# ApsaraDB/galaxysql

Measured on AMD Instinct MI355X. Metric: probe_rows_per_s, higher is better.
Workload: dtype int64; 1 GPU; C3_tpch_sf100_q3_join_chain_groupby; customer_rows_per_gpu=15000000, orders_rows_per_gpu=150000000, lineitem_rows_scanned_per_gpu=600000000, lineitem_rows_joined_per_gpu=323601457, groups_last_step=12883243, aggregates=SUM(revenue) f64 + SUM(rev_scaled4) i64 + COUNT(*), exchange=none, parallelism=hash_shuffle_dp1, probe_launches=81

## Files before the change

galaxysql_amd/abi.py:

```python
from __future__ import annotations

import ctypes as C
import os

import numpy as np

from .chunk import (Block, Chunk, I64, I32, F64, SLICE, DECIMAL,
                    _NP_DTYPES)

_REPO = os.path.dirname(os.path.dirname(os.path.abspath(__file__)))


class GxBlock(C.Structure):
    _fields_ = [
        ("type", C.c_int32),
        ("mem", C.c_int32),
        ("values", C.c_void_p),
        ("nulls", C.c_void_p),
        ("offsets", C.c_void_p),
        ("data", C.c_void_p),
        ("data_len", C.c_int64),
    ]


# ... 322 lines not shown
        L.gxop_window_close.argtypes = [C.c_void_p]
        L.gxop_fwindow_create.restype = C.c_void_p
        L.gxop_fwindow_create.argtypes = [C.POINTER(GxFWindowCfg)]
        L.gxop_fwindow_consume.argtypes = [C.c_void_p, C.POINTER(GxChunk)]
        L.gxop_fwindow_finish.argtypes = [C.c_void_p]
        L.gxop_fwindow_next.argtypes = [C.c_void_p,
                                        C.POINTER(C.POINTER(GxResult))]
        L.gxop_fwindow_close.argtypes = [C.c_void_p]
        L.gxop_part_create.restype = C.c_void_p
        L.gxop_part_create.argtypes = [C.POINTER(GxPartCfg)]
        L.gxop_part_consume.argtypes = [C.c_void_p, C.POINTER(GxChunk),
                                        C.POINTER(C.POINTER(GxResult))]
        L.gxop_part_consume_concat.argtypes = [C.c_void_p, C.POINTER(GxChunk),
                                               C.POINTER(C.POINTER(GxResult)),
                                               C.POINTER(C.c_int64)]
        L.gxop_part_close.argtypes = [C.c_void_p]
        L.gxop_scan_create.restype = C.c_void_p
        L.gxop_scan_create.argtypes = [C.POINTER(GxScanCfg)]
        L.gxop_scan_consume.argtypes = [C.c_void_p, C.POINTER(GxChunk),
                                        C.POINTER(C.POINTER(GxResult))]
        L.gxop_scan_close.argtypes = [C.c_void_p]
        self.has_probe_scan = hasattr(L, "gxop_join_probe_scan")
        if self.has_probe_scan:
            L.gxop_join_probe_scan.argtypes = [
                C.c_void_p, C.c_void_p, C.POINTER(GxChunk),
                C.POINTER(C.POINTER(GxResult)), C.POINTER(C.c_int64)]
        self.has_groupjoin_probe_scan = hasattr(L, "gxop_groupjoin_probe_scan")
        if self.has_groupjoin_probe_scan:
            L.gxop_groupjoin_probe_scan.argtypes = [
                C.c_void_p, C.c_void_p, C.POINTER(GxChunk),
                C.POINTER(C.c_int64), C.POINTER(C.c_int64)]
            L.gxop_groupjoin_get_stats.argtypes = [C.c_void_p,
                                                   C.POINTER(GxJoinStats)]
        self.has_sort = hasattr(L, "gxop_sort_create")
        if self.has_sort:
            L.gxop_sort_create.restype = C.c_void_p
            L.gxop_sort_create.argtypes = [C.POINTER(GxSortCfg)]
            L.gxop_sort_consume.argtypes = [C.c_void_p, C.POINTER(GxChunk)]
            L.gxop_sort_build.argtypes = [C.c_void_p]
            L.gxop_sort_next.argtypes = [C.c_void_p,
                                         C.POINTER(C.POINTER(GxResult))]
            L.gxop_sort_get_stats.argtypes = [C.c_void_p,
                                              C.POINTER(GxSortStats)]
            L.gxop_sort_close.restype = None
            L.gxop_sort_close.argtypes = [C.c_void_p]
        L.gxop_result_copy_col.argtypes = [C.POINTER(GxResult), C.c_int32,
                                           C.c_void_p, C.c_void_p]
        L.gxop_join_get_stats.argtypes = [C.c_void_p, C.POINTER(GxJoinStats)]
        L.gxop_agg_get_stats.argtypes = [C.c_void_p, C.POINTER(GxAggStats)]
        L.gxop_result_to_host.argtypes = [C.POINTER(GxResult)]
        L.gxop_result_release.argtypes = [C.POINTER(GxResult)]
        L.gx_last_error.restype = C.c_char_p
        L.gxop_abi_version.restype = C.c_int

    def error(self):
        return (self.lib.gx_last_error() or b"").decode()

    def check(self, rc, what):
        if rc != 0:
            raise RuntimeError(f"{what} failed (rc={rc}): {self.error()}")


    def to_gx_chunk(self, chunk: Chunk, keepalive, mem=0, device_ptrs=None):
        n = len(chunk.blocks) if chunk is not None else len(device_ptrs)
        blocks = (GxBlock * n)()
        if chunk is not None:
# ... 87 lines not shown
```

galaxysql_amd/csrc/gxhip.hip:

```cpp
#include "gx_common.h"
#include "gx_dec128.h"

#include <algorithm>
#include <cstdlib>
#include <deque>
#include <memory>
#include <mutex>
#include <hipcub/hipcub.hpp>

thread_local std::string gx_err;


#define GX_MAX_KEYS 4
#define GX_MAX_COLS 16

struct KeyViews {
    int32_t n;
    DevColView col[GX_MAX_KEYS];
};


#define XXP1 0x9E3779B185EBCA87ull
#define XXP2 0xC2B2AE3D27D4EB4Full
#define XXP3 0x165667B19E3779F9ull
// ... 271 lines not shown

struct JoinSpill {
    uint32_t row;
    uint32_t rank;
};

struct JoinInsertParams {
    DevColView key0;
    const int32_t *hashes;
    const uint8_t *keynull;
    int fast_i64;
    int64_t n;
    uint32_t mask;
    JoinEntry *table;
    JoinSpill *spill;
    uint32_t *spill_count;
    unsigned long long *bloom;
    uint32_t bloom_mask;
};

__device__ static inline uint32_t join_row_bucket(const JoinInsertParams &P,
                                                  int64_t i, int64_t &key) {
    int32_t h;
    if (P.fast_i64) {
        key = ((const int64_t *)P.key0.values)[i];
        h = gx_hash_i64(key);
    } else {
        h = P.hashes[i];
        key = (int64_t)h;
    }
    return (uint32_t)gx_mix(h) & P.mask;
}

__global__ void k_join_insert(JoinInsertParams P) {
    const int lane = threadIdx.x & 63;
    const int64_t stride = (int64_t)gridDim.x * blockDim.x;
    for (int64_t i = blockIdx.x * (int64_t)blockDim.x + threadIdx.x;;
         i += stride) {
        bool live = i < P.n;
        if (!__ballot(live)) break;
        if (live)
            live = P.fast_i64 ? !col_is_null(P.key0, i) : !P.keynull[i];
        uint32_t rank = 0;
        if (live) {
            int64_t key;
            uint32_t b = join_row_bucket(P, i, key);
            JoinEntry *bucket = P.table + (uint64_t)b * 4;
            rank = atomicAdd(&bucket[0].pad, 1u);
            if (rank < 4) {
                bucket[rank].key = key;
                bucket[rank].pos = (uint32_t)i;
            }
            if (P.bloom) {
                uint64_t x = bloom_mix(key);
                atomicOr(&P.bloom[bloom_word(x, P.bloom_mask)],
                         (unsigned long long)bloom_bits(x));
            }
        }
        bool spilled = live && rank >= 4;
        unsigned long long m = __ballot(spilled);
        if (m) {
            int leader = __ffsll((long long)m) - 1;
            uint32_t base = 0;
            if (lane == leader)
                base = atomicAdd(P.spill_count, (uint32_t)__popcll(m));
            base = (uint32_t)__shfl((int)base, leader, 64);
            if (spilled) {
                JoinSpill s;
                s.row = (uint32_t)i;
                s.rank = rank;
                P.spill[base + (uint32_t)__popcll(m & ((1ull << lane) - 1ull))] = s;
            }
        }
    }
}

__global__ void k_join_spill_reserve(JoinInsertParams P, uint32_t n_spill,
                                     uint32_t *cursor) {
    const int lane = threadIdx.x & 63;
    const int64_t stride = (int64_t)gridDim.x * blockDim.x;
    for (int64_t s = blockIdx.x * (int64_t)blockDim.x + threadIdx.x;;
         s += stride) {
        bool live = s < (int64_t)n_spill;
        if (!__ballot(live)) break;
        uint32_t want = 0;
        JoinEntry *bucket = nullptr;
        if (live && P.spill[s].rank == 4) {
            int64_t key;
            uint32_t b = join_row_bucket(P, P.spill[s].row, key);
            bucket = P.table + (uint64_t)b * 4;
            want = bucket[0].pad - 4;
        }
        uint32_t incl = want;
        for (int off = 1; off < 64; off <<= 1) {
            uint32_t t = (uint32_t)__shfl_up((int)incl, off, 64);
            if (lane >= off) incl += t;
        }
        uint32_t total = (uint32_t)__shfl((int)incl, 63, 64);
        if (total) {
            uint32_t base = 0;
            if (lane == 0) base = atomicAdd(cursor, total);
            base = (uint32_t)__shfl((int)base, 0, 64);
            if (want) bucket[1].pad = base + incl - want;
        }
    }
}
// ... 771 lines not shown
        if (conds.empty() || !d_cond_pats.empty()) return 0;
        d_cond_pats.resize(conds.size());
        for (size_t t = 0; t < conds.size(); t++) {
            const gx_join_cond &c = conds[t];
            if (c.col_b < 0 && c.v_bytes && c.v_len > 0) {
                if (d_cond_pats[t].grow((size_t)c.v_len, stream)) return -1;
                HIP_OK(hipMemcpyAsync(d_cond_pats[t].p, c.v_bytes,
                                      (size_t)c.v_len, hipMemcpyHostToDevice,
                                      stream));
            }
        }
        return 0;
    }

    KeyViews key_views(const DevStore &s, const std::vector<int> &colidx) const {
        KeyViews kv;
        kv.n = (int32_t)colidx.size();
        for (int i = 0; i < kv.n; i++) kv.col[i] = s.view(colidx[i]);
        return kv;
    }
    KeyViews key_views_staged(const StagedChunk &s, const std::vector<int> &colidx) const {
        KeyViews kv;
        kv.n = (int32_t)colidx.size();
        for (int i = 0; i < kv.n; i++) kv.col[i] = s.views[colidx[i]];
        return kv;
    }

    int consume(const gx_chunk *ch) {
        if (ensure_device(device)) return -1;
        return build.append(ch);
    }

    int do_build() {
        if (built) return 0;
        if (ensure_device(device)) return -1;
        const int64_t n = build.n_rows;
        fast_i64 = (keys.size() == 1 && keys[0].unified_type == GX_I64)
                   && !null_safe_keys;

        bool semi_join = (cfg.join_type == GX_JOIN_SEMI || cfg.join_type == GX_JOIN_ANTI)
                         && !cfg.single_join;
        if (n == 0 && cfg.join_type == GX_JOIN_INNER) pass_nothing = true;
        if (semi_join && n == 0) {
            if (cfg.join_type == GX_JOIN_SEMI) pass_nothing = true;
            else pass_through = true;
        }

        if (n == 0) {
            n_buckets = 2;
            mask = 1;
            if (null_safe_keys) {
                if (d_starts.grow((size_t)(n_buckets + 1) * 4, stream)) return -1;
                HIP_OK(hipMemsetAsync(d_starts.p, 0, (size_t)(n_buckets + 1) * 4, stream));
            } else {
                if (d_table.grow((size_t)n_buckets * 4 * sizeof(JoinEntry),
                                 stream)) return -1;
                HIP_OK(hipMemsetAsync(d_table.p, 0,
                                      (size_t)n_buckets * 4 * sizeof(JoinEntry),
                                      stream));
            }
        }
        if (n > 0 && null_safe_keys) {
            if (d_hashes.grow((size_t)n * 4, stream) ||
                d_keynull.grow((size_t)n, stream)) return -1;
            KeyViews bk = key_views(build, build_key_cols);
            hipLaunchKernelGGL(k_hash_rows, dim3(gx_grid(n)), dim3(256), 0, stream,
// ... 37 lines not shown
            HIP_OK(hipMemsetAsync(d_counts.p, 0, 8, stream));
            if (!fast_i64) {
                if (d_hashes.grow((size_t)n * 4, stream) ||
                    d_keynull.grow((size_t)n, stream)) return -1;
                hipLaunchKernelGGL(k_hash_rows, dim3(gx_grid(n)), dim3(256), 0,
                                   stream, key_views(build, build_key_cols), n,
                                   (int32_t *)d_hashes.p, (uint8_t *)d_keynull.p,
                                   0);
            }
            const char *be = getenv("GX_BLOOM");
            bool use_bloom = fast_i64 &&
                (be ? be[0] == '1'
                    : (cfg.enable_bloom == 1 && n >= (1 << 16) &&
                       n <= INT64_C(200) << 20));
            if (use_bloom) {
                int64_t n_lines = gx_pow2(std::max<int64_t>(n / 64, 1));
                bloom_mask = (uint32_t)(n_lines - 1);
                if (d_bloom.grow((size_t)n_lines * 64, stream)) return -1;
                HIP_OK(hipMemsetAsync(d_bloom.p, 0, (size_t)n_lines * 64,
                                      stream));
            }
            JoinInsertParams IP;
            IP.key0 = build.view(build_key_cols[0]);
            IP.hashes = (const int32_t *)d_hashes.p;
            IP.keynull = (const uint8_t *)d_keynull.p;
            IP.fast_i64 = (int)fast_i64;
            IP.n = n;
            IP.mask = mask;
            IP.table = (JoinEntry *)d_table.p;
            IP.spill = (JoinSpill *)d_spill.p;
            IP.spill_count = (uint32_t *)d_counts.p;
            IP.bloom = use_bloom ? (unsigned long long *)d_bloom.p : nullptr;
            IP.bloom_mask = bloom_mask;
            hipLaunchKernelGGL(k_join_insert, dim3(gx_grid(n)), dim3(256), 0,
                               stream, IP);
            uint32_t n_spill = 0;
            HIP_OK(hipMemcpyAsync(&n_spill, d_counts.p, 4,
                                  hipMemcpyDeviceToHost, stream));
            HIP_OK(hipStreamSynchronize(stream));
            if (d_entries.grow((size_t)std::max<uint32_t>(n_spill, 1) *
                                   sizeof(JoinEntry), stream)) return -1;
            if (n_spill > 0) {
                hipLaunchKernelGGL(k_join_spill_reserve, dim3(gx_grid(n_spill)),
                                   dim3(256), 0, stream, IP, n_spill,
                                   (uint32_t *)d_counts.p + 1);
                hipLaunchKernelGGL(k_join_spill_place, dim3(gx_grid(n_spill)),
                                   dim3(256), 0, stream, IP, n_spill,
                                   (JoinEntry *)d_entries.p);
            }
        }

        if (cfg.join_type == GX_JOIN_ANTI && cfg.anti_null_col >= 0 &&
            build.cols.size() == 1 && n > 0 && build.cols[0].has_nulls) {
            DevBuf flag;
            if (flag.grow(4, stream)) return -1;
            HIP_OK(hipMemsetAsync(flag.p, 0, 4, stream));
            hipLaunchKernelGGL(k_any_null, dim3(gx_grid(n)), dim3(256), 0, stream,
                               build.view(0), n, (uint32_t *)flag.p);
            uint32_t f = 0;
            HIP_OK(hipMemcpyAsync(&f, flag.p, 4, hipMemcpyDeviceToHost, stream));
            HIP_OK(hipStreamSynchronize(stream));
            if (f) pass_nothing = true;
        }

        if (cfg.build_outer) {
            size_t words = (size_t)((n + 31) / 32);
            if (words == 0) words = 1;
            if (d_bitmap.grow(words * 4, stream)) return -1;
// ... 554 lines not shown
```

galaxysql_amd/csrc/gxhip_groupjoin.inc:

```

namespace {

struct __align__(16) GJWideEntry {
    int64_t key;
    uint32_t pos;
    uint32_t used;
    unsigned long long s[2];
};

__global__ void k_gjw_expand(const JoinEntry *entries, int64_t n,
                             DevColView keycol, GJWideEntry *wide,
                             unsigned long long s0, unsigned long long s1) {
    for (int64_t i = blockIdx.x * (int64_t)blockDim.x + threadIdx.x; i < n;
         i += (int64_t)gridDim.x * blockDim.x) {
        JoinEntry e = entries[i];
        GJWideEntry w;
        w.key = ((const int64_t *)keycol.values)[e.pos];
        w.pos = e.pos;
        w.used = 0;
        w.s[0] = s0;
        w.s[1] = s1;
        wide[i] = w;
    }
}
// ... 270 lines not shown
                ((int64_t *)P.agg_vals[a])[i] = (int64_t)v +
                    ((!matched && P.count_row_null_row) ? 1 : 0);
            } else {
                ((unsigned long long *)P.agg_vals[a])[i] = v;
            }
        }
    }
}

struct GroupJoinOp : gx_op {
    gx_groupjoin_cfg cfg;
    std::vector<gx_equi_key> keys;
    std::vector<int32_t> build_types, probe_types, group_cols_;
    std::vector<gx_agg_spec> aggs;

    DevBuf d_accum;
    DevBuf d_wide;
    DevBuf d_pn, d_ph, d_gj_tmp, d_cnt, d_gidx, d_used, d_records;
    DevBuf d_meta;
    std::unique_ptr<JoinOp> jop;
    hipEvent_t ev0 = nullptr, ev1 = nullptr;
    double kernel_ms = 0.0;
    int64_t rows_total = 0, probe_launches = 0, matches_total = 0;
    int32_t stride = 0;
    int32_t val_off[GX_MAX_COLS] = {0};
    int32_t seen_off[GX_MAX_COLS] = {0};
    unsigned long long tmpl[2 * GX_MAX_COLS] = {0};
    bool built = false, emitted = false;
    bool wide_ok = false;
    bool wide = false;
    bool inline_ok = false;
    bool inline_tab = false;
    int32_t count_off = -1;

    GroupJoinOp(const gx_groupjoin_cfg *c)
        : gx_op(OP_GROUPJOIN, c->device, c->stream), cfg(*c) {
        keys.assign(c->keys, c->keys + c->n_keys);
        build_types.assign(c->build_types, c->build_types + c->n_build_cols);
        probe_types.assign(c->probe_types, c->probe_types + c->n_probe_cols);
        group_cols_.assign(c->group_cols, c->group_cols + c->n_group_cols);
        aggs.assign(c->aggs, c->aggs + c->n_aggs);

        gx_join_cfg jc{};
        jc.join_type = GX_JOIN_INNER;
        jc.n_keys = (int32_t)keys.size();
        swapped_keys = keys;
        for (auto &k : swapped_keys) std::swap(k.outer_index, k.inner_index);
        jc.keys = swapped_keys.data();
        jc.n_outer_cols = (int32_t)probe_types.size();
        jc.outer_types = probe_types.data();
        jc.n_inner_cols = (int32_t)build_types.size();
        jc.inner_types = build_types.data();
        jc.anti_null_col = -1;
        jc.device = device;
        jc.stream = (uint64_t)stream;
        jc.expected_build_rows = c->expected_build_rows;
        jc.enable_bloom = 1;
        jop.reset(new JoinOp(&jc));
        jop->null_safe_keys = true;

        int32_t off = 0;
        for (size_t a = 0; a < aggs.size(); a++) {
            val_off[a] = off;
            switch (aggs[a].func) {
            case GX_AGG_MIN_I64: tmpl[off] = (unsigned long long)INT64_MAX; break;
            case GX_AGG_MAX_I64: tmpl[off] = (unsigned long long)INT64_MIN; break;
// ... 9 lines not shown
                                 aggs[a].func == GX_AGG_BIT_AND ||
                                 aggs[a].func == GX_AGG_BIT_OR ||
                                 aggs[a].func == GX_AGG_BIT_XOR);
            if (tracks_null) {
                seen_off[a] = off;
                tmpl[off] = 0ull;
                off++;
            } else {
                seen_off[a] = -1;
            }
        }
        stride = off > 0 ? off : 1;
        wide_ok = keys.size() == 1 && keys[0].unified_type == GX_I64 &&
                  aggs.size() <= 2;
        for (auto &a : aggs)
            wide_ok &= a.func == GX_AGG_COUNT_ROW ||
                       a.func == GX_AGG_COUNT_COL ||
                       a.func == GX_AGG_SUM_I64;
        inline_ok = !wide_ok && keys.size() == 1 &&
                    keys[0].unified_type == GX_I64 &&
                    build_types[keys[0].outer_index] == GX_I64 &&
                    probe_types[keys[0].inner_index] == GX_I64;
    }
    std::vector<gx_equi_key> swapped_keys;

    ~GroupJoinOp() override {
        if (ev0) (void)hipEventDestroy(ev0);
        if (ev1) (void)hipEventDestroy(ev1);
    }

    int consume(const gx_chunk *ch) { return jop->consume(ch); }

    int do_build() {
        inline_tab = inline_ok && jop->build.n_rows > 0 &&
                     !jop->build.cols[jop->build_key_cols[0]].has_nulls;
        jop->null_safe_keys = !inline_tab;
        count_off = -1;
        if (inline_tab && cfg.join_type == GX_JOIN_INNER)
            for (size_t a = 0; a < aggs.size() && count_off < 0; a++)
                if (aggs[a].func == GX_AGG_COUNT_ROW) count_off = val_off[a];
        if (jop->do_build()) return -1;
        const int64_t n = jop->build.n_rows;
        if (d_meta.grow(16, stream)) return -1;
        HIP_OK(hipMemsetAsync(d_meta.p, 0, 16, stream));
        if (n > 0) {
            if (d_records.grow((size_t)n * stride * 8, stream)) return -1;
            AggInitParams P;
            P.records = (unsigned long long *)d_records.p;
            P.stride = stride;
            P.from = 0;
            P.to = n;
            std::memcpy(P.tmpl, tmpl, sizeof(tmpl));
            hipLaunchKernelGGL(k_agg_init, dim3(gx_grid(n * stride)),
                               dim3(256), 0, stream, P);
        }
        size_t words = (size_t)((n + 31) / 32);
        if (words == 0) words = 1;
        if (d_used.grow(words * 4, stream)) return -1;
        HIP_OK(hipMemsetAsync(d_used.p, 0, words * 4, stream));
        wide = wide_ok && n > 0 &&
               !jop->build.cols[jop->build_key_cols[0]].has_nulls;
        if (wide) {
            if (d_wide.grow((size_t)n * sizeof(GJWideEntry), stream))
                return -1;
            hipLaunchKernelGGL(k_gjw_expand, dim3(gx_grid(n)), dim3(256), 0,
                               stream, (const JoinEntry *)jop->d_entries.p, n,
                               jop->build.view(jop->build_key_cols[0]),
                               (GJWideEntry *)d_wide.p, tmpl[val_off[0]],
                               aggs.size() > 1 ? tmpl[val_off[1]] : 0ull);
        }
        built = true;
        return 0;
    }

// ... 302 lines not shown
```

galaxysql_amd/csrc/gxhip_scan.inc:

```

namespace {

#define GX_MAX_PREDS 8

struct ScanPreds {
    int32_t n_preds;
    int32_t pred_cmp[GX_MAX_PREDS];
    int64_t pred_i64[GX_MAX_PREDS];
    double  pred_f64[GX_MAX_PREDS];
    const uint8_t *pred_pat[GX_MAX_PREDS];
    int32_t pred_plen[GX_MAX_PREDS];
    DevColView pred_view[GX_MAX_PREDS];
};

struct ScanParams {
    int64_t n;
    ScanPreds preds;
    int32_t n_projs;
    int32_t proj_op[GX_MAX_COLS];
    int32_t proj_scale[GX_MAX_COLS];
    DevColView proj_a[GX_MAX_COLS];
    DevColView proj_b[GX_MAX_COLS];
    DevColView proj_c[GX_MAX_COLS];
    DevColView proj_d[GX_MAX_COLS];
// ... 469 lines not shown
    AccumFlush flush;
    flush.A = A;
    probe_scan_body(P, S, kept, flush);
}

struct ProjGatherParams {
    const uint32_t *pidx;
    const uint32_t *bidx;
    int64_t n;
    int32_t n_cols;
    int32_t side[GX_MAX_COLS];
    int32_t op[GX_MAX_COLS];
    int32_t scale[GX_MAX_COLS];
    DevColView a[GX_MAX_COLS];
    DevColView b[GX_MAX_COLS];
    DevColView c[GX_MAX_COLS];
    DevColView d[GX_MAX_COLS];
    void *out_vals[GX_MAX_COLS];
    uint8_t *out_nulls[GX_MAX_COLS];
};

__global__ void k_gather_proj(ProjGatherParams G) {
    for (int64_t i = blockIdx.x * (int64_t)blockDim.x + threadIdx.x; i < G.n;
         i += (int64_t)gridDim.x * blockDim.x) {
        const int64_t pi = G.pidx[i];
        const int64_t bi = G.bidx[i];
        for (int c = 0; c < G.n_cols; c++)
            proj_store(G.op[c], G.scale[c], G.a[c], G.b[c], G.c[c], G.d[c],
                       G.side[c] ? bi : pi, G.out_vals[c], G.out_nulls[c], i,
                       nullptr);
    }
}

__global__ void k_scan(ScanParams P) {
    __shared__ uint32_t s_rows[4][GX_EMIT_STAGE];
    const int wid = threadIdx.x >> 6;
    const int lane = threadIdx.x & 63;
    uint32_t *stage = s_rows[wid];
    uint32_t cnt = 0;

    auto flush = [&]() {
        if (cnt == 0) return;
        uint32_t base = 0;
        if (lane == 0) base = atomicAdd(P.counter, cnt);
        base = (uint32_t)__shfl((int)base, 0, 64);
        for (uint32_t k = (uint32_t)lane; k < cnt; k += 64) {
            uint32_t at = base + k;
            if (at >= P.cap) continue;
            int64_t src = stage[k];
            if (P.out_rowids) P.out_rowids[at] = (uint32_t)src;
            for (int c = 0; c < P.n_projs; c++)
                proj_store(P.proj_op[c], P.proj_scale[c], P.proj_a[c],
                           P.proj_b[c], P.proj_c[c], P.proj_d[c], src,
                           P.out_vals[c], P.out_nulls[c], at, P.err);
        }
        cnt = 0;
    };

    const int64_t stride = (int64_t)gridDim.x * blockDim.x;
    for (int64_t base_i = blockIdx.x * (int64_t)blockDim.x + threadIdx.x;;
         base_i += stride) {
        bool active = base_i < P.n;
        if (!__ballot(active)) break;
        bool want = active && scan_row_passes(P.preds, base_i);
        unsigned long long m = __ballot(want);
        uint32_t add = (uint32_t)__popcll(m);
// ... 140 lines not shown
                return -1;
        }
        give_result(std::move(h), out);
        return 0;
    }
};


bool probe_scan_fast_ok(const JoinOp *j, const ScanOp *s,
                        const gx_chunk *raw) {
    if (!j->built || !j->fast_i64 || j->pass_nothing || j->pass_through)
        return false;
    const gx_join_cfg &c = j->cfg;
    if (c.build_outer || c.single_join || !j->conds.empty()) return false;
    if (c.join_type != GX_JOIN_INNER && c.join_type != GX_JOIN_SEMI)
        return false;
    if (raw->n_rows <= 0 || raw->n_blocks != (int32_t)s->input_types.size())
        return false;
    for (int32_t b = 0; b < raw->n_blocks; b++)
        if (raw->blocks[b].mem != GX_MEM_DEVICE) return false;
    const gx_proj &kp = s->projs[(size_t)j->probe_key_cols[0]];
    if (kp.op != GX_PROJ_COPY || s->input_types[kp.a] != GX_I64) return false;
    for (size_t p = 0; p < s->projs.size(); p++)
        if (s->projs[p].op == GX_PROJ_DEC_TO_SCALED ||
            s->out_types[p] == GX_SLICE)
            return false;
    std::vector<JoinOp::OutSpec> specs = j->projected_specs();
    if (specs.size() > GX_MAX_COLS) return false;
    for (auto &sp : specs)
        if (sp.type == GX_SLICE) return false;
    return true;
}

int probe_scan_fused(JoinOp *j, ScanOp *s, const gx_chunk *raw,
                     gx_result **out, int64_t *n_kept) {
    if (ensure_device(j->device)) return -1;
    hipStream_t stream = j->stream;
    StagedChunk st;
    if (st.stage(raw, stream)) return -1;
    const int64_t n = st.n_rows;
    ScanPreds S;
    if (s->fill_preds(S, st)) return -1;
    const gx_proj &kp = s->projs[(size_t)j->probe_key_cols[0]];

    uint32_t cap = (uint32_t)std::min<int64_t>(
        std::max<int64_t>((int64_t)n * 2, 1 << 16), INT64_C(1) << 31);
    if (j->d_meta.grow(16, stream)) return -1;
    for (int attempt = 0; attempt < 4; attempt++) {
        if (j->d_pidx.grow((size_t)cap * 4, stream) ||
            j->d_bpos.grow((size_t)cap * 4, stream)) return -1;
        HIP_OK(hipMemsetAsync(j->d_meta.p, 0, 16, stream));
        ProbeParams P;
        std::memset(&P, 0, sizeof(P));
        P.table = (const JoinEntry *)j->d_table.p;
        P.entries = (const JoinEntry *)j->d_entries.p;
        P.mask = j->mask;
        P.n_probe = n;
        P.bloom = (const uint32_t *)j->d_bloom.p;
        P.bloom_mask = j->bloom_mask;
        P.fast_i64 = 1;
        P.build_keys = j->key_views(j->build, j->build_key_cols);
        P.probe_keys.n = 1;
        P.probe_keys.col[0] = st.views[kp.a];
        P.join_type = j->cfg.join_type;
        P.semi_join = j->cfg.join_type == GX_JOIN_SEMI;
        P.anti_null_col = -1;
        P.out_probe = (uint32_t *)j->d_pidx.p;
        P.out_build = (uint32_t *)j->d_bpos.p;
        P.cap = cap;
        P.counter = (uint32_t *)j->d_meta.p;
        P.err = (uint32_t *)j->d_meta.p + 1;
        if (!j->ev0) {
            HIP_OK(hipEventCreate(&j->ev0));
            HIP_OK(hipEventCreate(&j->ev1));
        }
        HIP_OK(hipEventRecord(j->ev0, stream));
        hipLaunchKernelGGL(k_probe_scan, dim3(gx_ps_grid(n)), dim3(256), 0,
                           stream, P, S, (uint32_t *)j->d_meta.p + 2);
        HIP_OK(hipEventRecord(j->ev1, stream));
        uint32_t meta[3];
        HIP_OK(hipMemcpyAsync(meta, j->d_meta.p, 12, hipMemcpyDeviceToHost,
                              stream));
        HIP_OK(hipStreamSynchronize(stream));
        {
            float ms = 0;
            HIP_OK(hipEventElapsedTime(&ms, j->ev0, j->ev1));
            j->probe_kernel_ms += ms;
            j->probe_launches++;
        }
        if (meta[0] > cap) { cap = meta[0]; continue; }

        const int64_t n_out = meta[0];
        j->probe_rows_total += meta[2];
        j->matches_total += n_out;
        *n_kept = meta[2];
        std::vector<JoinOp::OutSpec> specs = j->projected_specs();
        std::vector<int32_t> otypes;
        std::vector<uint8_t> null_free;
        for (auto &sp : specs) {
            otypes.push_back(sp.type);
            null_free.push_back(sp.outer
                ? s->proj_null_free((size_t)sp.src, st)
                : !j->build.view(sp.src).has_nulls);
        }
        auto h = alloc_result_cols(otypes, n_out, j->device, stream,
                                   &null_free);
        if (!h) return -1;
        if (n_out > 0) {
            ProjGatherParams G;
            std::memset(&G, 0, sizeof(G));
            G.pidx = (const uint32_t *)j->d_pidx.p;
            G.bidx = (const uint32_t *)j->d_bpos.p;
            G.n = n_out;
            G.n_cols = (int32_t)specs.size();
            for (size_t c = 0; c < specs.size(); c++) {
                G.out_vals[c] = h->bufs[c * 2].p;
                G.out_nulls[c] = (uint8_t *)h->bufs[c * 2 + 1].p;
                if (!specs[c].outer) {
                    G.side[c] = 1;
                    G.op[c] = GX_PROJ_COPY;
                    G.a[c] = j->build.view(specs[c].src);
                    continue;
                }
                const gx_proj &pr = s->projs[(size_t)specs[c].src];
                G.side[c] = 0;
                G.op[c] = pr.op;
                G.a[c] = st.views[pr.a];
                if (pr.op == GX_PROJ_SCALED_TO_DEC)
                    G.scale[c] = pr.c;
                else if (pr.op != GX_PROJ_COPY)
                    G.b[c] = st.views[pr.b];
                if (pr.op == GX_PROJ_Q9_AMOUNT4) {
                    G.c[c] = st.views[pr.c];
                    G.d[c] = st.views[pr.d];
                }
            }
            hipLaunchKernelGGL(k_gather_proj, dim3(gx_grid(n_out)), dim3(256),
                               0, stream, G);
            HIP_OK(hipStreamSynchronize(stream));
        }
        give_result(std::move(h), out);
        return 0;
    }
    return -1;
}


bool gj_probe_scan_fast_ok(const GroupJoinOp *g, const ScanOp *s,
                           const gx_chunk *raw) {
    if (!g->inline_tab || g->jop->pass_nothing) return false;
    if (raw->n_rows <= 0 || (int64_t)raw->n_rows >= (INT64_C(1) << 31) ||
        raw->n_blocks != (int32_t)s->input_types.size())
        return false;
    for (int32_t b = 0; b < raw->n_blocks; b++)
        if (raw->blocks[b].mem != GX_MEM_DEVICE) return false;
    const gx_proj &kp = s->projs[(size_t)g->jop->probe_key_cols[0]];
    if (kp.op != GX_PROJ_COPY || s->input_types[kp.a] != GX_I64) return false;
    for (auto &pr : s->projs)
        if (pr.op == GX_PROJ_DEC_TO_SCALED) return false;
    for (auto &sp : g->aggs) {
        if (sp.input_col < 0) continue;
        const gx_proj &pr = s->projs[(size_t)sp.input_col];
        const int32_t t = s->out_types[(size_t)sp.input_col];
        switch (pr.op) {
        case GX_PROJ_COPY:
            if (t != GX_I64 && t != GX_I32 && t != GX_F64) return false;
            break;
        case GX_PROJ_REV_F64: case GX_PROJ_REV_SCALED4:
        case GX_PROJ_Q9_AMOUNT4:
            break;
        default:
            return false;
        }
    }
    return true;
}

// ... 41 lines not shown
            A.d[a] = st.views[pr.d];
        }
    }
    bool additive = g->stride <= GX_AGG_T_SLOTS;
    for (size_t a = 0; a < g->aggs.size(); a++)
        additive = additive && agg_func_additive(g->aggs[a].func);
    if (additive) {
        A.t_width = g->stride <= 1 ? 1 : g->stride == 2 ? 2 : 4;
        for (size_t a = 0; a < g->aggs.size(); a++)
            if (agg_func_adds_f64(g->aggs[a].func))
                A.t_f64 |= 1u << g->val_off[a];
    }
    A.records = (unsigned long long *)g->d_records.p;
    A.used = g->count_off >= 0 ? nullptr : (uint32_t *)g->d_used.p;
    A.matches = (unsigned long long *)g->d_meta.p;
    if (g->d_accum.grow(sizeof(A), stream)) return -1;
    HIP_OK(hipMemcpyAsync(g->d_accum.p, &A, sizeof(A), hipMemcpyHostToDevice,
                          stream));
    HIP_OK(hipMemsetAsync((char *)g->d_meta.p + 8, 0, 4, stream));
    if (!g->ev0) {
        HIP_OK(hipEventCreate(&g->ev0));
        HIP_OK(hipEventCreate(&g->ev1));
    }
    HIP_OK(hipEventRecord(g->ev0, stream));
    hipLaunchKernelGGL(k_gj_probe_scan, dim3(gx_ps_grid(n)), dim3(256), 0,
                       stream, P, S, (uint32_t *)g->d_meta.p + 2,
                       (const GJAccum *)g->d_accum.p);
    HIP_OK(hipEventRecord(g->ev1, stream));
    if (g->finish_probe(n_kept)) return -1;
    g->rows_total += *n_kept;
    return 0;
}

}

extern "C" {

int gxop_groupjoin_probe_scan(gx_op *groupjoin, gx_op *scan,
                              const gx_chunk *raw_chunk,
                              int64_t *n_scan_kept, int64_t *n_matched) {
    if (!groupjoin || groupjoin->kind != OP_GROUPJOIN) { gx_set_err("not a groupjoin op"); return -1; }
    if (!scan || scan->kind != OP_SCAN) { gx_set_err("not a scan op"); return -1; }
    if (!raw_chunk) { gx_set_err("groupjoin_probe_scan: null argument"); return -1; }
    if (groupjoin->device != scan->device || groupjoin->stream != scan->stream) {
        gx_set_err("groupjoin_probe_scan: group-join and scan must share "
                   "device and stream");
        return -1;
    }
    GroupJoinOp *g = static_cast<GroupJoinOp *>(groupjoin);
    ScanOp *s = static_cast<ScanOp *>(scan);
    std::lock_guard<std::mutex> lk(groupjoin->mu);
    if (g->probe_types != s->out_types) {
        gx_set_err("groupjoin_probe_scan: scan's projected types differ "
                   "from the group-join's probe_types");
        return -1;
    }
    if (!g->built) { gx_set_err("probe before build"); return -1; }
    const int64_t before = g->matches_total;
    int64_t kept = 0;
    int rc;
    if (gj_probe_scan_fast_ok(g, s, raw_chunk)) {
        rc = gj_probe_scan_fused(g, s, raw_chunk, &kept);
    } else {
        gx_result *t = nullptr;
        rc = s->consume(raw_chunk, &t);
        if (rc) return rc;
        kept = t->chunk.n_rows;
        rc = g->probe(&t->chunk);
        gxop_result_release(t);
// ... 84 lines not shown
```

galaxysql_amd/operators.py:

```python
from __future__ import annotations

import ctypes as C

from . import abi
from .abi import (GxJoinCfg, GxEquiKey, GxAggCfg, GxAggSpec, GxPartCfg, GxResult)
from .chunk import Chunk, CHUNK_SIZE


class EquiJoinKey:

    def __init__(self, outer_index, inner_index, unified_type):
        self.outer_index = outer_index
        self.inner_index = inner_index
        self.unified_type = unified_type


class JoinCond:

    def __init__(self, col_a, cmp, col_b=-1, value=None):
        self.col_a = col_a
        self.cmp = cmp
        self.col_b = col_b
        self.value = value

# ... 300 lines not shown
        self._lib = lib
        self._keep = []
        keys = (GxEquiKey * len(join_keys))()
        for i, k in enumerate(join_keys):
            keys[i] = GxEquiKey(k.outer_index, k.inner_index, k.unified_type, 0)
        bt = (C.c_int32 * len(build_types))(*build_types)
        pt = (C.c_int32 * len(probe_types))(*probe_types)
        gc = (C.c_int32 * max(1, len(group_cols)))(*(group_cols or [0]))
        sp = (GxAggSpec * max(1, len(aggs)))()
        for i, (f, col) in enumerate(aggs):
            sp[i] = GxAggSpec(f, col)
        cfg = GxGroupJoinCfg(
            join_type=join_type, n_keys=len(join_keys), keys=keys,
            n_build_cols=len(build_types), build_types=bt,
            n_probe_cols=len(probe_types), probe_types=pt,
            n_group_cols=len(group_cols), group_cols=gc,
            n_aggs=len(aggs), aggs=sp, device=device, stream=stream,
            expected_build_rows=expected_build_rows)
        self._keep += [keys, bt, pt, gc, sp, cfg]
        self._op = lib.lib.gxop_groupjoin_create(C.byref(cfg))
        if not self._op:
            raise RuntimeError(f"gxop_groupjoin_create: {lib.error()}")

    def consume_chunk(self, chunk: Chunk):
        ka = []
        gc = self._lib.to_gx_chunk(chunk, ka)
        self._lib.check(
            self._lib.lib.gxop_groupjoin_consume(self._op, C.byref(gc)),
            "groupjoin_consume")

    def build_consume(self):
        self._lib.check(self._lib.lib.gxop_groupjoin_build(self._op),
                        "groupjoin_build")

    def probe_chunk(self, chunk: Chunk):
        ka = []
        gc = self._lib.to_gx_chunk(chunk, ka)
        self._lib.check(
            self._lib.lib.gxop_groupjoin_probe(self._op, C.byref(gc)),
            "groupjoin_probe")

    def probe_scan(self, scan, chunk_ref):
        kept = C.c_int64(0)
        matched = C.c_int64(0)
        self._lib.check(self._lib.lib.gxop_groupjoin_probe_scan(
            self._op, scan._op, chunk_ref, C.byref(kept), C.byref(matched)),
            "groupjoin_probe_scan")
        return kept.value, matched.value

    def stats(self):
        from .abi import GxJoinStats
        s = GxJoinStats()
        self._lib.check(
            self._lib.lib.gxop_groupjoin_get_stats(self._op, C.byref(s)),
            "groupjoin_get_stats")
        return {"probe_kernel_ms": s.probe_kernel_ms,
                "probe_launches": s.probe_launches,
                "probe_rows": s.probe_rows, "matches": s.matches}

    def result_chunks(self):
        chunks = []
        while True:
            out = C.POINTER(GxResult)()
            self._lib.check(
                self._lib.lib.gxop_groupjoin_next(self._op, C.byref(out)),
                "groupjoin_next")
# ... 290 lines not shown
```

galaxysql_amd/queries.py:

```python
from __future__ import annotations

import ctypes as C

from . import abi
from .abi import GxResult
from .chunk import I64, I32, F64, SLICE
from .exchange import chunk_from_torch
from .operators import (ParallelHashJoinExec, HashAggExec, HashGroupJoinExec,
                        EquiJoinKey)

CUST_TYPES = [I64]
ORDERS_TYPES = [I64, I64, I32, I32]
LINEITEM_TYPES = [I64, F64, I64]
Q3_RESULT_TYPES = [I64, I32, I32, F64, I64, I64]


def _consume_tensors(lib, op, tensors, types):
    ka = []
    gc = chunk_from_torch(lib, tensors, types, ka)
    lib.check(lib.lib.gxop_join_consume(op._op, C.byref(gc)), "join_consume")


def _probe_tensors(lib, op, tensors, types):
    ka = []
# ... 35 lines not shown

def _src_rows(src):
    if isinstance(src, list):
        return src[0].numel()
    return src.contents.chunk.n_rows


_TORCH_DT = None


def _torch_dtypes():
    global _TORCH_DT
    if _TORCH_DT is None:
        import torch
        _TORCH_DT = {I64: torch.int64, I32: torch.int32, F64: torch.float64}
    return _TORCH_DT


def result_to_tensors(lib, res, types, device_t):
    import torch
    n = res.contents.chunk.n_rows
    dt = _torch_dtypes()
    cols = []
    for ci, ty in enumerate(types):
        t = torch.empty(n, dtype=dt[ty], device=device_t)
        if n:
            lib.check(lib.lib.gxop_result_copy_col(
                res, ci, C.c_void_p(t.data_ptr()), None), "result_copy_col")
        cols.append(t)
    return cols


def _q3_groupjoin(lib, device, r1, n_orders_kept, lineitem, to_host,
                  keep_results):
    gj = HashGroupJoinExec(
        lib, abi.INNER, [EquiJoinKey(1, 0, I64)],
        build_types=ORDERS_TYPES, probe_types=LINEITEM_TYPES,
        group_cols=[1, 2, 3],
        aggs=[(abi.SUM_F64, 1), (abi.SUM_I64, 2), (abi.COUNT_ROW, -1)],
        device=device, expected_build_rows=n_orders_kept)
    try:
        if r1:
            lib.check(lib.lib.gxop_groupjoin_consume(
                gj._op, C.byref(r1.contents.chunk)), "groupjoin_consume")
        gj.build_consume()
        if r1:
            lib.lib.gxop_result_release(r1)
            r1 = None
        lineitem.kept, n_joined = gj.probe_scan(lineitem.scan,
                                                C.byref(lineitem.chunk))
        j2_stats = gj.stats()
        if to_host:
            chunks = gj.result_chunks()
            n_groups = sum(c.n_rows for c in chunks)
        else:
            chunks = []
            n_groups = 0
            while True:
                out = C.POINTER(GxResult)()
                lib.check(lib.lib.gxop_groupjoin_next(gj._op, C.byref(out)),
                          "groupjoin_next")
                if not out:
                    break
                n_groups += out.contents.chunk.n_rows
                if keep_results is not None:
                    keep_results.append(out)
                else:
                    lib.lib.gxop_result_release(out)
        info = {"orders_kept": n_orders_kept, "joined_rows": n_joined,
                "groups": n_groups, "join2_stats": j2_stats}
        return chunks, info
    finally:
        if r1:
            lib.lib.gxop_result_release(r1)
        gj.close()


def run_q3(lib, device, cust, orders, lineitem, expected_groups=0,
           to_host=True, reshuffle_by_orderkey=False, local_rank=0,
           keep_results=None):
    j1 = ParallelHashJoinExec(
        lib, abi.SEMI, [EquiJoinKey(0, 0, I64)],
        outer_types=ORDERS_TYPES, inner_types=CUST_TYPES,
        device=device, expected_build_rows=_src_rows(cust),
        enable_bloom=True)
    try:
        _consume_src(lib, j1, cust, CUST_TYPES)
        j1.build_consume()
        r1 = _probe_src(lib, j1, orders, ORDERS_TYPES)
        n_orders_kept = r1.contents.chunk.n_rows if r1 else 0

        if (isinstance(lineitem, _ScanSrc) and not reshuffle_by_orderkey
                and getattr(lib, "has_groupjoin_probe_scan", False)):
            return _q3_groupjoin(lib, device, r1, n_orders_kept, lineitem,
                                 to_host, keep_results)

        j2 = ParallelHashJoinExec(
            lib, abi.INNER, [EquiJoinKey(0, 1, I64)],
            outer_types=LINEITEM_TYPES, inner_types=ORDERS_TYPES,
            device=device, expected_build_rows=n_orders_kept,
            out_proj=[0, 1, 2, 5, 6],
            enable_bloom=True)
        try:
            if reshuffle_by_orderkey:
                from .exchange import shuffle_columns
                cols = result_to_tensors(lib, r1, ORDERS_TYPES,
                                         cust[0].device) if r1 else None
                if r1:
                    lib.lib.gxop_result_release(r1)
                    r1 = None
                cols = shuffle_columns(lib, cols, ORDERS_TYPES, [1],
                                       device=device)
                n_orders_kept = cols[0].numel()
                _consume_tensors(lib, j2, cols, ORDERS_TYPES)
            elif r1:
                lib.check(lib.lib.gxop_join_consume(
                    j2._op, C.byref(r1.contents.chunk)), "join_consume")
            j2.build_consume()
            if r1:
                lib.lib.gxop_result_release(r1)
                r1 = None
# ... 562 lines not shown
```

include/gxop_hip.h:

```cpp
#ifndef GXOP_HIP_H
#define GXOP_HIP_H

#include "gxop.h"

#ifdef __cplusplus
extern "C" {
#endif


int gxop_join_probe_scan(gx_op *join, gx_op *scan, const gx_chunk *raw_chunk,
                         gx_result **out, int64_t *n_scan_kept);


int gxop_groupjoin_probe_scan(gx_op *groupjoin, gx_op *scan,
                              const gx_chunk *raw_chunk,
                              int64_t *n_scan_kept, int64_t *n_matched);

int gxop_groupjoin_get_stats(gx_op *groupjoin, gx_join_stats *out);


typedef struct gx_order_by {
    int32_t col;
    int32_t asc;
    int32_t null_last;
} gx_order_by;

typedef struct gx_sort_cfg {
    int32_t n_cols;
    const int32_t *types;
    int32_t n_order;
    const gx_order_by *order;
    int64_t offset;
    int64_t fetch;
    int64_t expected_rows;
    int64_t compact_rows;
    int32_t out_chunk_rows;
    int32_t device;
    uint64_t stream;
} gx_sort_cfg;

typedef struct gx_sort_stats {
    int64_t rows_consumed;
    int64_t rows_kept;
    int64_t compactions;
    int32_t used_select;
    int32_t select_passes;
    int64_t candidates;
    double kernel_ms;
} gx_sort_stats;
// ... 13 lines not shown
```

Before: 21.36 billion rows/s.

## Fuse orders semi-join projection directly into groupjoin hash-table build

Adds a fused path in which the customer-orders semi-join probe writes its projected columns straight into the groupjoin's build store, and the hash insert happens in the same kernel (k_join_insert_proj). This avoids materialising an intermediate result, copying it into the groupjoin build store, and launching a separate gather kernel. The change also refactors the probe-scan into reusable pieces and adds an env-var opt-out with a fallback to the old path. The metric counts lineitem probe rows, so build-side savings may barely move it.

```diff
diff --git a/galaxysql_amd/abi.py b/galaxysql_amd/abi.py
--- a/galaxysql_amd/abi.py
+++ b/galaxysql_amd/abi.py
@@ -378,6 +378,13 @@
                 C.POINTER(C.c_int64), C.POINTER(C.c_int64)]
             L.gxop_groupjoin_get_stats.argtypes = [C.c_void_p,
                                                    C.POINTER(GxJoinStats)]
+        self.has_groupjoin_build_probe_scan = hasattr(
+            L, "gxop_groupjoin_build_probe_scan")
+        if self.has_groupjoin_build_probe_scan:
+            L.gxop_groupjoin_build_probe_scan.argtypes = [
+                C.c_void_p, C.c_void_p, C.c_void_p, C.POINTER(GxChunk),
+                C.POINTER(C.c_int64), C.POINTER(C.c_int64)]
+            L.gxop_groupjoin_build_was_fused.argtypes = [C.c_void_p]
         self.has_sort = hasattr(L, "gxop_sort_create")
         if self.has_sort:
             L.gxop_sort_create.restype = C.c_void_p
diff --git a/galaxysql_amd/csrc/gxhip.hip b/galaxysql_amd/csrc/gxhip.hip
--- a/galaxysql_amd/csrc/gxhip.hip
+++ b/galaxysql_amd/csrc/gxhip.hip
@@ -327,6 +327,41 @@
     return (uint32_t)gx_mix(h) & P.mask;
 }
 
+__device__ static inline void join_insert_row(const JoinInsertParams &P,
+                                              bool live, int64_t key,
+                                              uint32_t b, int64_t i,
+                                              int lane) {
+    uint32_t rank = 0;
+    if (live) {
+        JoinEntry *bucket = P.table + (uint64_t)b * 4;
+        rank = atomicAdd(&bucket[0].pad, 1u);
+        if (rank < 4) {
+            bucket[rank].key = key;
+            bucket[rank].pos = (uint32_t)i;
+        }
+        if (P.bloom) {
+            uint64_t x = bloom_mix(key);
+            atomicOr(&P.bloom[bloom_word(x, P.bloom_mask)],
+                     (unsigned long long)bloom_bits(x));
+        }
+    }
+    bool spilled = live && rank >= 4;
+    unsigned long long m = __ballot(spilled);
+    if (m) {
+        int leader = __ffsll((long long)m) - 1;
+        uint32_t base = 0;
+        if (lane == leader)
+            base = atomicAdd(P.spill_count, (uint32_t)__popcll(m));
+        base = (uint32_t)__shfl((int)base, leader, 64);
+        if (spilled) {
+            JoinSpill s;
+            s.row = (uint32_t)i;
+            s.rank = rank;
+            P.spill[base + (uint32_t)__popcll(m & ((1ull << lane) - 1ull))] = s;
+        }
+    }
+}
+
 __global__ void k_join_insert(JoinInsertParams P) {
     const int lane = threadIdx.x & 63;
     const int64_t stride = (int64_t)gridDim.x * blockDim.x;
@@ -336,37 +371,10 @@
         if (!__ballot(live)) break;
         if (live)
             live = P.fast_i64 ? !col_is_null(P.key0, i) : !P.keynull[i];
-        uint32_t rank = 0;
-        if (live) {
-            int64_t key;
-            uint32_t b = join_row_bucket(P, i, key);
-            JoinEntry *bucket = P.table + (uint64_t)b * 4;
-            rank = atomicAdd(&bucket[0].pad, 1u);
-            if (rank < 4) {
-                bucket[rank].key = key;
-                bucket[rank].pos = (uint32_t)i;
-            }
-            if (P.bloom) {
-                uint64_t x = bloom_mix(key);
-                atomicOr(&P.bloom[bloom_word(x, P.bloom_mask)],
-                         (unsigned long long)bloom_bits(x));
-            }
-        }
-        bool spilled = live && rank >= 4;
-        unsigned long long m = __ballot(spilled);
-        if (m) {
-            int leader = __ffsll((long long)m) - 1;
-            uint32_t base = 0;
-            if (lane == leader)
-                base = atomicAdd(P.spill_count, (uint32_t)__popcll(m));
-            base = (uint32_t)__shfl((int)base, leader, 64);
-            if (spilled) {
-                JoinSpill s;
-                s.row = (uint32_t)i;
-                s.rank = rank;
-                P.spill[base + (uint32_t)__popcll(m & ((1ull << lane) - 1ull))] = s;
-            }
-        }
+        int64_t key = 0;
+        uint32_t b = 0;
+        if (live) b = join_row_bucket(P, i, key);
+        join_insert_row(P, live, key, b, i, lane);
     }
 }
 
@@ -1204,6 +1212,14 @@
     }
 
     int do_build() {
+        return do_build_with([this](const JoinInsertParams &IP) {
+            hipLaunchKernelGGL(k_join_insert, dim3(gx_grid(IP.n)), dim3(256),
+                               0, stream, IP);
+        });
+    }
+
+    template <class LaunchInsert>
+    int do_build_with(LaunchInsert &&launch_insert) {
         if (built) return 0;
         if (ensure_device(device)) return -1;
         const int64_t n = build.n_rows;
@@ -1307,8 +1323,7 @@
             IP.spill_count = (uint32_t *)d_counts.p;
             IP.bloom = use_bloom ? (unsigned long long *)d_bloom.p : nullptr;
             IP.bloom_mask = bloom_mask;
-            hipLaunchKernelGGL(k_join_insert, dim3(gx_grid(n)), dim3(256), 0,
-                               stream, IP);
+            launch_insert(IP);
             uint32_t n_spill = 0;
             HIP_OK(hipMemcpyAsync(&n_spill, d_counts.p, 4,
                                   hipMemcpyDeviceToHost, stream));
diff --git a/galaxysql_amd/csrc/gxhip_groupjoin.inc b/galaxysql_amd/csrc/gxhip_groupjoin.inc
--- a/galaxysql_amd/csrc/gxhip_groupjoin.inc
+++ b/galaxysql_amd/csrc/gxhip_groupjoin.inc
@@ -326,6 +326,7 @@
     bool inline_ok = false;
     bool inline_tab = false;
     int32_t count_off = -1;
+    bool build_fused = false;
 
     GroupJoinOp(const gx_groupjoin_cfg *c)
         : gx_op(OP_GROUPJOIN, c->device, c->stream), cfg(*c) {
@@ -401,6 +402,14 @@
     int consume(const gx_chunk *ch) { return jop->consume(ch); }
 
     int do_build() {
+        return do_build_with([this](const JoinInsertParams &IP) {
+            hipLaunchKernelGGL(k_join_insert, dim3(gx_grid(IP.n)), dim3(256),
+                               0, stream, IP);
+        });
+    }
+
+    template <class LaunchInsert>
+    int do_build_with(LaunchInsert &&launch_insert) {
         inline_tab = inline_ok && jop->build.n_rows > 0 &&
                      !jop->build.cols[jop->build_key_cols[0]].has_nulls;
         jop->null_safe_keys = !inline_tab;
@@ -408,7 +417,7 @@
         if (inline_tab && cfg.join_type == GX_JOIN_INNER)
             for (size_t a = 0; a < aggs.size() && count_off < 0; a++)
                 if (aggs[a].func == GX_AGG_COUNT_ROW) count_off = val_off[a];
-        if (jop->do_build()) return -1;
+        if (jop->do_build_with(launch_insert)) return -1;
         const int64_t n = jop->build.n_rows;
         if (d_meta.grow(16, stream)) return -1;
         HIP_OK(hipMemsetAsync(d_meta.p, 0, 16, stream));
diff --git a/galaxysql_amd/csrc/gxhip_scan.inc b/galaxysql_amd/csrc/gxhip_scan.inc
--- a/galaxysql_amd/csrc/gxhip_scan.inc
+++ b/galaxysql_amd/csrc/gxhip_scan.inc
@@ -525,6 +525,51 @@
     }
 }
 
+#define GX_JIP_MAX_COLS 8
+
+__global__ void __launch_bounds__(256)
+k_join_insert_proj(JoinInsertParams P, ProjGatherParams G, int32_t key_col) {
+    const int lane = threadIdx.x & 63;
+    const int64_t stride = (int64_t)gridDim.x * blockDim.x;
+    for (int64_t i = blockIdx.x * (int64_t)blockDim.x + threadIdx.x;;
+         i += stride) {
+        const bool live = i < P.n;
+        if (!__ballot(live)) break;
+        unsigned long long val[GX_JIP_MAX_COLS];
+        uint32_t nullm = 0;
+        int64_t key = 0;
+        if (live) {
+            const int64_t pi = G.pidx[i];
+            const int64_t bi = G.bidx[i];
+#pragma unroll
+            for (int c = 0; c < GX_JIP_MAX_COLS; c++) {
+                val[c] = 0;
+                if (c < G.n_cols) {
+                    const AggVal v = proj_value(G.op[c], G.a[c], G.b[c],
+                                                G.c[c], G.d[c],
+                                                G.side[c] ? bi : pi);
+                    val[c] = v.bits;
+                    if (v.isnull) nullm |= 1u << c;
+                }
+            }
+#pragma unroll
+            for (int c = 0; c < GX_JIP_MAX_COLS; c++) {
+                if (c < G.n_cols) {
+                    if (G.out_nulls[c])
+                        G.out_nulls[c][i] = (uint8_t)((nullm >> c) & 1u);
+                    if (G.op[c] == GX_PROJ_COPY && G.a[c].type == GX_I32)
+                        ((int32_t *)G.out_vals[c])[i] = (int32_t)val[c];
+                    else
+                        ((unsigned long long *)G.out_vals[c])[i] = val[c];
+                    if (c == key_col) key = (int64_t)val[c];
+                }
+            }
+        }
+        const uint32_t b = (uint32_t)gx_mix(gx_hash_i64(key)) & P.mask;
+        join_insert_row(P, live, key, b, i, lane);
+    }
+}
+
 __global__ void k_scan(ScanParams P) {
     __shared__ uint32_t s_rows[4][GX_EMIT_STAGE];
     const int wid = threadIdx.x >> 6;
@@ -731,12 +776,9 @@
     return true;
 }
 
-int probe_scan_fused(JoinOp *j, ScanOp *s, const gx_chunk *raw,
-                     gx_result **out, int64_t *n_kept) {
-    if (ensure_device(j->device)) return -1;
+int probe_scan_pairs(JoinOp *j, ScanOp *s, const StagedChunk &st,
+                     int64_t *n_out, int64_t *n_kept) {
     hipStream_t stream = j->stream;
-    StagedChunk st;
-    if (st.stage(raw, stream)) return -1;
     const int64_t n = st.n_rows;
     ScanPreds S;
     if (s->fill_preds(S, st)) return -1;
@@ -789,59 +831,85 @@
         }
         if (meta[0] > cap) { cap = meta[0]; continue; }
 
-        const int64_t n_out = meta[0];
+        *n_out = meta[0];
         j->probe_rows_total += meta[2];
-        j->matches_total += n_out;
+        j->matches_total += meta[0];
         *n_kept = meta[2];
-        std::vector<JoinOp::OutSpec> specs = j->projected_specs();
-        std::vector<int32_t> otypes;
-        std::vector<uint8_t> null_free;
-        for (auto &sp : specs) {
-            otypes.push_back(sp.type);
-            null_free.push_back(sp.outer
-                ? s->proj_null_free((size_t)sp.src, st)
-                : !j->build.view(sp.src).has_nulls);
-        }
-        auto h = alloc_result_cols(otypes, n_out, j->device, stream,
-                                   &null_free);
-        if (!h) return -1;
-        if (n_out > 0) {
-            ProjGatherParams G;
-            std::memset(&G, 0, sizeof(G));
-            G.pidx = (const uint32_t *)j->d_pidx.p;
-            G.bidx = (const uint32_t *)j->d_bpos.p;
-            G.n = n_out;
-            G.n_cols = (int32_t)specs.size();
-            for (size_t c = 0; c < specs.size(); c++) {
-                G.out_vals[c] = h->bufs[c * 2].p;
-                G.out_nulls[c] = (uint8_t *)h->bufs[c * 2 + 1].p;
-                if (!specs[c].outer) {
-                    G.side[c] = 1;
-                    G.op[c] = GX_PROJ_COPY;
-                    G.a[c] = j->build.view(specs[c].src);
-                    continue;
-                }
-                const gx_proj &pr = s->projs[(size_t)specs[c].src];
-                G.side[c] = 0;
-                G.op[c] = pr.op;
-                G.a[c] = st.views[pr.a];
-                if (pr.op == GX_PROJ_SCALED_TO_DEC)
-                    G.scale[c] = pr.c;
-                else if (pr.op != GX_PROJ_COPY)
-                    G.b[c] = st.views[pr.b];
-                if (pr.op == GX_PROJ_Q9_AMOUNT4) {
-                    G.c[c] = st.views[pr.c];
-                    G.d[c] = st.views[pr.d];
-                }
-            }
-            hipLaunchKernelGGL(k_gather_proj, dim3(gx_grid(n_out)), dim3(256),
-                               0, stream, G);
-            HIP_OK(hipStreamSynchronize(stream));
-        }
-        give_result(std::move(h), out);
         return 0;
     }
+    gx_set_err("probe_scan: pair list still short after 4 resizes");
     return -1;
+}
+
+void fill_proj_gather(ProjGatherParams &G, const JoinOp *j, const ScanOp *s,
+                      const StagedChunk &st,
+                      const std::vector<JoinOp::OutSpec> &specs,
+                      int64_t n_out) {
+    G.pidx = (const uint32_t *)j->d_pidx.p;
+    G.bidx = (const uint32_t *)j->d_bpos.p;
+    G.n = n_out;
+    G.n_cols = (int32_t)specs.size();
+    for (size_t c = 0; c < specs.size(); c++) {
+        if (!specs[c].outer) {
+            G.side[c] = 1;
+            G.op[c] = GX_PROJ_COPY;
+            G.a[c] = j->build.view(specs[c].src);
+            continue;
+        }
+        const gx_proj &pr = s->projs[(size_t)specs[c].src];
+        G.side[c] = 0;
+        G.op[c] = pr.op;
+        G.a[c] = st.views[pr.a];
+        if (pr.op == GX_PROJ_SCALED_TO_DEC)
+            G.scale[c] = pr.c;
+        else if (pr.op != GX_PROJ_COPY)
+            G.b[c] = st.views[pr.b];
+        if (pr.op == GX_PROJ_Q9_AMOUNT4) {
+            G.c[c] = st.views[pr.c];
+            G.d[c] = st.views[pr.d];
+        }
+    }
+}
+
+bool probe_scan_col_null_free(const JoinOp *j, const ScanOp *s,
+                              const StagedChunk &st,
+                              const JoinOp::OutSpec &sp) {
+    return sp.outer ? s->proj_null_free((size_t)sp.src, st)
+                    : !j->build.view(sp.src).has_nulls;
+}
+
+int probe_scan_fused(JoinOp *j, ScanOp *s, const gx_chunk *raw,
+                     gx_result **out, int64_t *n_kept) {
+    if (ensure_device(j->device)) return -1;
+    hipStream_t stream = j->stream;
+    StagedChunk st;
+    if (st.stage(raw, stream)) return -1;
+    int64_t n_out = 0;
+    if (probe_scan_pairs(j, s, st, &n_out, n_kept)) return -1;
+
+    std::vector<JoinOp::OutSpec> specs = j->projected_specs();
+    std::vector<int32_t> otypes;
+    std::vector<uint8_t> null_free;
+    for (auto &sp : specs) {
+        otypes.push_back(sp.type);
+        null_free.push_back(probe_scan_col_null_free(j, s, st, sp));
+    }
+    auto h = alloc_result_cols(otypes, n_out, j->device, stream, &null_free);
+    if (!h) return -1;
+    if (n_out > 0) {
+        ProjGatherParams G;
+        std::memset(&G, 0, sizeof(G));
+        fill_proj_gather(G, j, s, st, specs, n_out);
+        for (size_t c = 0; c < specs.size(); c++) {
+            G.out_vals[c] = h->bufs[c * 2].p;
+            G.out_nulls[c] = (uint8_t *)h->bufs[c * 2 + 1].p;
+        }
+        hipLaunchKernelGGL(k_gather_proj, dim3(gx_grid(n_out)), dim3(256),
+                           0, stream, G);
+        HIP_OK(hipStreamSynchronize(stream));
+    }
+    give_result(std::move(h), out);
+    return 0;
 }
 
 
@@ -949,9 +1017,138 @@
     return 0;
 }
 
+
+bool gj_build_probe_scan_fast_ok(const GroupJoinOp *g, const JoinOp *j,
+                                 const ScanOp *s, const gx_chunk *raw,
+                                 const StagedChunk &st) {
+    const char *e = getenv("GX_GJ_BUILD_FUSED");
+    if (e && e[0] == '0') return false;
+    if (!probe_scan_fast_ok(j, s, raw)) return false;
+    if (g->built || g->jop->built || g->jop->build.n_rows != 0 ||
+        !g->inline_ok)
+        return false;
+    if (g->device != j->device || g->stream != j->stream) return false;
+    const std::vector<JoinOp::OutSpec> specs = j->projected_specs();
+    if (specs.size() > GX_JIP_MAX_COLS) return false;
+    for (size_t c = 0; c < specs.size(); c++) {
+        const JoinOp::OutSpec &sp = specs[c];
+        if (sp.type != GX_I64 && sp.type != GX_I32 && sp.type != GX_F64)
+            return false;
+        if (sp.outer && s->projs[(size_t)sp.src].op == GX_PROJ_SCALED_TO_DEC)
+            return false;
+    }
+    const int kc = g->jop->build_key_cols[0];
+    return probe_scan_col_null_free(j, s, st, specs[(size_t)kc]);
+}
+
+int gj_store_size_exact(DevStore &store, int64_t n,
+                        const std::vector<uint8_t> &null_free) {
+    if (store.reserve(n)) return -1;
+    for (size_t c = 0; c < store.cols.size(); c++) {
+        DevColumn &col = store.cols[c];
+        col.has_nulls = !null_free[c];
+        if (col.has_nulls && col.nulls.grow((size_t)n, store.stream))
+            return -1;
+    }
+    store.n_rows = n;
+    return 0;
+}
+
+int gj_build_probe_scan_fused(GroupJoinOp *g, JoinOp *j, ScanOp *s,
+                              const StagedChunk &st, int64_t *n_kept,
+                              int64_t *n_consumed) {
+    hipStream_t stream = j->stream;
+    int64_t n = 0;
+    if (probe_scan_pairs(j, s, st, &n, n_kept)) return -1;
+    *n_consumed = n;
+    if (n == 0) return g->do_build();
+
+    const std::vector<JoinOp::OutSpec> specs = j->projected_specs();
+    std::vector<uint8_t> null_free;
+    for (auto &sp : specs)
+        null_free.push_back(probe_scan_col_null_free(j, s, st, sp));
+    DevStore &store = g->jop->build;
+    if (gj_store_size_exact(store, n, null_free)) return -1;
+
+    ProjGatherParams G;
+    std::memset(&G, 0, sizeof(G));
+    fill_proj_gather(G, j, s, st, specs, n);
+    for (size_t c = 0; c < specs.size(); c++) {
+        G.out_vals[c] = store.cols[c].values.p;
+        G.out_nulls[c] = store.cols[c].has_nulls
+            ? (uint8_t *)store.cols[c].nulls.p : nullptr;
+    }
+    const int32_t key_col = (int32_t)g->jop->build_key_cols[0];
+    g->build_fused = true;
+    return g->do_build_with([&](const JoinInsertParams &IP) {
+        hipLaunchKernelGGL(k_join_insert_proj, dim3(gx_grid(IP.n)), dim3(256),
+                           0, stream, IP, G, key_col);
+    });
+}
+
 }
 
 extern "C" {
+
+int gxop_groupjoin_build_probe_scan(gx_op *groupjoin, gx_op *join,
+                                    gx_op *scan, const gx_chunk *raw_chunk,
+                                    int64_t *n_scan_kept,
+                                    int64_t *n_consumed) {
+    if (!groupjoin || groupjoin->kind != OP_GROUPJOIN) { gx_set_err("not a groupjoin op"); return -1; }
+    if (!join || join->kind != OP_JOIN) { gx_set_err("not a join op"); return -1; }
+    if (!scan || scan->kind != OP_SCAN) { gx_set_err("not a scan op"); return -1; }
+    if (!raw_chunk) { gx_set_err("groupjoin_build_probe_scan: null argument"); return -1; }
+    GroupJoinOp *g = static_cast<GroupJoinOp *>(groupjoin);
+    ScanOp *s = static_cast<ScanOp *>(scan);
+    JoinOp *j = join->variant == 0 ? static_cast<JoinOp *>(join) : nullptr;
+    int64_t kept = 0, consumed = 0;
+    {
+        std::unique_lock<std::mutex> lj(join->mu, std::defer_lock);
+        std::unique_lock<std::mutex> lg(groupjoin->mu, std::defer_lock);
+        std::lock(lj, lg);
+        if (g->built) { gx_set_err("groupjoin_build_probe_scan: already built"); return -1; }
+        const bool shape_ok = j && j->built &&
+            (j->cfg.build_outer ? j->inner_types : j->outer_types) ==
+                s->out_types &&
+            j->output_types() == g->build_types &&
+            join->device == scan->device && join->stream == scan->stream;
+        if (shape_ok) {
+            if (ensure_device(j->device)) return -1;
+            StagedChunk st;
+            bool fast = true;
+            for (int32_t b = 0; b < raw_chunk->n_blocks && fast; b++)
+                fast = raw_chunk->blocks[b].mem == GX_MEM_DEVICE;
+            if (fast && st.stage(raw_chunk, j->stream)) return -1;
+            if (fast && gj_build_probe_scan_fast_ok(g, j, s, raw_chunk, st)) {
+                int rc = gj_build_probe_scan_fused(g, j, s, st, &kept,
+                                                   &consumed);
+                if (rc) return rc;
+                if (n_scan_kept) *n_scan_kept = kept;
+                if (n_consumed) *n_consumed = consumed;
+                return 0;
+            }
+        }
+    }
+    gx_result *t = nullptr;
+    int rc = gxop_join_probe_scan(join, scan, raw_chunk, &t, &kept);
+    if (rc) return rc;
+    if (t) {
+        consumed = t->chunk.n_rows;
+        rc = gxop_groupjoin_consume(groupjoin, &t->chunk);
+        gxop_result_release(t);
+        if (rc) return rc;
+    }
+    rc = gxop_groupjoin_build(groupjoin);
+    if (rc) return rc;
+    if (n_scan_kept) *n_scan_kept = kept;
+    if (n_consumed) *n_consumed = consumed;
+    return 0;
+}
+
+int gxop_groupjoin_build_was_fused(gx_op *groupjoin) {
+    if (!groupjoin || groupjoin->kind != OP_GROUPJOIN) { gx_set_err("not a groupjoin op"); return -1; }
+    return static_cast<GroupJoinOp *>(groupjoin)->build_fused ? 1 : 0;
+}
 
 int gxop_groupjoin_probe_scan(gx_op *groupjoin, gx_op *scan,
                               const gx_chunk *raw_chunk,
diff --git a/galaxysql_amd/operators.py b/galaxysql_amd/operators.py
--- a/galaxysql_amd/operators.py
+++ b/galaxysql_amd/operators.py
@@ -356,6 +356,17 @@
     def build_consume(self):
         self._lib.check(self._lib.lib.gxop_groupjoin_build(self._op),
                         "groupjoin_build")
+
+    def build_probe_scan(self, join, scan, chunk_ref):
+        kept = C.c_int64(0)
+        consumed = C.c_int64(0)
+        self._lib.check(self._lib.lib.gxop_groupjoin_build_probe_scan(
+            self._op, join._op, scan._op, chunk_ref, C.byref(kept),
+            C.byref(consumed)), "groupjoin_build_probe_scan")
+        return kept.value, consumed.value
+
+    def build_was_fused(self):
+        return self._lib.lib.gxop_groupjoin_build_was_fused(self._op) == 1
 
     def probe_chunk(self, chunk: Chunk):
         ka = []
diff --git a/galaxysql_amd/queries.py b/galaxysql_amd/queries.py
--- a/galaxysql_amd/queries.py
+++ b/galaxysql_amd/queries.py
@@ -91,7 +91,7 @@
 
 
 def _q3_groupjoin(lib, device, r1, n_orders_kept, lineitem, to_host,
-                  keep_results):
+                  keep_results, producer=None):
     gj = HashGroupJoinExec(
         lib, abi.INNER, [EquiJoinKey(1, 0, I64)],
         build_types=ORDERS_TYPES, probe_types=LINEITEM_TYPES,
@@ -99,10 +99,15 @@
         aggs=[(abi.SUM_F64, 1), (abi.SUM_I64, 2), (abi.COUNT_ROW, -1)],
         device=device, expected_build_rows=n_orders_kept)
     try:
-        if r1:
-            lib.check(lib.lib.gxop_groupjoin_consume(
-                gj._op, C.byref(r1.contents.chunk)), "groupjoin_consume")
-        gj.build_consume()
+        if producer is not None:
+            j1, orders = producer
+            orders.kept, n_orders_kept = gj.build_probe_scan(
+                j1, orders.scan, C.byref(orders.chunk))
+        else:
+            if r1:
+                lib.check(lib.lib.gxop_groupjoin_consume(
+                    gj._op, C.byref(r1.contents.chunk)), "groupjoin_consume")
+            gj.build_consume()
         if r1:
             lib.lib.gxop_result_release(r1)
             r1 = None
@@ -146,6 +151,12 @@
     try:
         _consume_src(lib, j1, cust, CUST_TYPES)
         j1.build_consume()
+        if (isinstance(orders, _ScanSrc) and isinstance(lineitem, _ScanSrc)
+                and not reshuffle_by_orderkey
+                and getattr(lib, "has_groupjoin_build_probe_scan", False)
+                and getattr(lib, "has_groupjoin_probe_scan", False)):
+            return _q3_groupjoin(lib, device, None, 0, lineitem, to_host,
+                                 keep_results, producer=(j1, orders))
         r1 = _probe_src(lib, j1, orders, ORDERS_TYPES)
         n_orders_kept = r1.contents.chunk.n_rows if r1 else 0
 
diff --git a/include/gxop_hip.h b/include/gxop_hip.h
--- a/include/gxop_hip.h
+++ b/include/gxop_hip.h
@@ -15,6 +15,14 @@
 int gxop_groupjoin_probe_scan(gx_op *groupjoin, gx_op *scan,
                               const gx_chunk *raw_chunk,
                               int64_t *n_scan_kept, int64_t *n_matched);
+
+
+int gxop_groupjoin_build_probe_scan(gx_op *groupjoin, gx_op *join,
+                                    gx_op *scan, const gx_chunk *raw_chunk,
+                                    int64_t *n_scan_kept,
+                                    int64_t *n_consumed);
+
+int gxop_groupjoin_build_was_fused(gx_op *groupjoin);
 
 int gxop_groupjoin_get_stats(gx_op *groupjoin, gx_join_stats *out);
 
```

Measured after the change: 22.59 billion rows/s (median of 6 runs). 1.06x the previous value.
